# gk969/stm32-speech-recognition

Hardware: AMD Instinct MI355X
Metric: utterances/sec (256-frame, 100 templates) (higher is better)
Workload: dtype int32

## Files before the change

include/sr_engine.h:

```cpp
#ifndef SR_ENGINE_H
#define SR_ENGINE_H

#include <stddef.h>
#include <stdint.h>

#ifdef __cplusplus
extern "C" {
#endif

#define SR_OK 0
#define SR_ERR_NO_DEVICE 1
#define SR_ERR_BAD_CONFIG 2
#define SR_ERR_BAD_ARG 3
#define SR_ERR_NO_TEMPLATES 4
#define SR_ERR_HIP 5

#define SR_ST_OK 0
#define SR_ST_VAD_FAIL 1
#define SR_ST_MFCC_FAIL 2
#define SR_ST_SEG_OOB 3

#define SR_DIS_ERR 0xFFFFFFFFu
#define SR_SAVE_MASK 12345u

// ... 35 lines not shown

typedef struct sr_engine sr_engine;

void sr_default_config(sr_config *cfg);
int sr_create(const sr_config *cfg, sr_engine **out);
void sr_destroy(sr_engine *h);
const char *sr_last_error(void);

typedef struct sr_tables {
    uint16_t *hamm;
    uint16_t *tri_cen;
    uint16_t *tri_even;
    uint16_t *tri_odd;
    int8_t *dct;
    int16_t *tw_kr;
    int16_t *tw_ki;
    uint32_t *log_thr;
} sr_tables;
int sr_build_tables(const sr_config *cfg, const sr_tables *out);
int sr_build_tie_table(int8_t *out);
int sr_log_table_mismatches(void);
uint32_t sr_mag_cheap_bound(const sr_engine *h);
uint32_t sr_mag_table(uint16_t *out, uint32_t n);

int sr_set_templates(sr_engine *h, const void *store, uint32_t n_slots, uint32_t stride_bytes);
int sr_set_templates_dense(sr_engine *h, const int16_t *mfcc, const uint32_t *frames, const uint8_t *valid,
                           uint32_t n_templates, uint32_t tpl_stride);
uint32_t sr_num_templates(const sr_engine *h);
int sr_train_store(sr_engine *h, const uint16_t *pcm, uint64_t pcm_stride, uint32_t buf_len, uint32_t n,
                   const uint32_t *slot, void *store, uint32_t n_slots, uint32_t stride_bytes, uint32_t *status);

int sr_recognize_batch(sr_engine *h, const uint16_t *pcm, uint64_t pcm_stride, uint32_t buf_len, uint32_t B,
                       sr_result *results, uint32_t *scores, int16_t *mfcc, sr_vad_rec *vad);
int sr_recognize_batch_dev(sr_engine *h, const uint16_t *d_pcm, uint64_t pcm_stride, uint32_t buf_len, uint32_t B,
                           sr_result *d_results, uint32_t *d_scores, int16_t *d_mfcc, sr_vad_rec *d_vad,
                           void *stream);
int sr_recognize_batch_packed12(sr_engine *h, const uint8_t *packed, uint64_t row_stride_bytes, uint32_t buf_len, uint32_t B,
                                sr_result *results, uint32_t *scores, int16_t *mfcc, sr_vad_rec *vad);

int sr_recognize_segments_batch(sr_engine *h, const uint16_t *pcm, uint64_t pcm_stride, uint32_t buf_len, uint32_t B,
                                sr_result *results, uint32_t *scores, sr_vad_rec *vad);
int sr_recognize_segments_batch_dev(sr_engine *h, const uint16_t *d_pcm, uint64_t pcm_stride, uint32_t buf_len,
                                    uint32_t B, sr_result *d_results, uint32_t *d_scores, sr_vad_rec *d_vad,
                                    void *stream);

typedef struct sr_stream_seg {
// ... 242 lines not shown
```

stm32_speech_recognition_amd/csrc/k_mfcc.hip:

```cpp
#include "sr_fft_dev.h"

#include <type_traits>

#ifndef SR_MEL_CHUNKED
#define SR_MEL_CHUNKED 1
#endif

namespace sr {

constexpr int kMfccWaves = 4;
constexpr int kFramesPerWave = 16, kFramesPerWaveMid = 4, kFramesPerWaveSmall = 1;
#ifndef SR_MAG_TAB_BINS
#define SR_MAG_TAB_BINS 8
#endif
constexpr int mfcc_tab_bins(int fpw) { return fpw == kFramesPerWave ? SR_MAG_TAB_BINS : 0; }
static_assert(SR_MAG_TAB_BINS == 0 || SR_MAG_TAB_BINS == 4 || SR_MAG_TAB_BINS == 8, "table bins per lane");
#ifndef SR_MFCC_PIPE
#define SR_MFCC_PIPE 1
#endif
#ifndef SR_MFCC_PIPE_PEEL
#define SR_MFCC_PIPE_PEEL 1
#endif
#ifndef SR_MFCC_PIPE_VMCNT
#define SR_MFCC_PIPE_VMCNT (SR_MFCC_PIPE_PEEL ? 3 : 0)
#endif
static_assert(SR_MFCC_PIPE_VMCNT == 0 || (SR_MFCC_PIPE_VMCNT == 3 && SR_MFCC_PIPE_PEEL), "younger loads counted by the wait");
constexpr bool mfcc_pipelined(int fpw) { return SR_MFCC_PIPE && mfcc_tab_bins(fpw) == 8; }
constexpr int kMelPad = kMel + 1;
__device__ __forceinline__ constexpr int mel_chunk_word(int j) { return 256 * ((j >> 2) & 1) + 4 * ((j >> 3) ^ (4 * ((j >> 2) & 1))) + (j & 3); }
constexpr int mfcc_wave_lds_words(int fpw) { return kXchgWords + fpw * kMelPad + 64; }

template <typename Base>
struct MfccTabArgs : Base {
    const uint16_t *mag_q;
    uint32_t mag_table_off;
};
template <typename Base>
constexpr int mfcc_feat_kind<MfccTabArgs<Base>> = mfcc_feat_kind<Base>;
template <typename Base>
static MfccTabArgs<Base> mfcc_tab_args(const Base &b, const MfccMagTab &tab)
{
    MfccTabArgs<Base> r;
    static_cast<Base &>(r) = b;
    r.mag_q = tab.mag_q;
    r.mag_table_off = tab.mag_table_off;
    return r;
}

template <int kFPW, typename Args = MfccTabArgs<MfccArgs>>
__global__ void __launch_bounds__(64 * kMfccWaves, 4) k_mfcc(const Args a)
{
    constexpr int kFeat = mfcc_feat_kind<Args>;
    constexpr uint32_t kFeatW = (kFeat == SR_FEAT_FFT || kFeat == SR_FEAT_MAG) ? kBins : kMel;
    constexpr int kWaveLdsWords = mfcc_wave_lds_words(kFPW);
    constexpr int kTabBins = mfcc_tab_bins(kFPW);
    constexpr bool kPipe = mfcc_pipelined(kFPW);
    extern __shared__ __attribute__((aligned(16))) uint32_t smem[];
    __shared__ uint32_t s_dctM[kCoef * kMelPad];
    __shared__ int s_dctS[kCoef * kMelPad];
    __shared__ u32x4 s_tw3[kTw3Row * 4], s_tw5[8 * 64];
    __shared__ u32x4 s_tm[4 * 64];
    const int lane = threadIdx.x & 63, w = __builtin_amdgcn_readfirstlane(threadIdx.x >> 6);
    uint32_t *buf = smem + w * kWaveLdsWords;
    uint32_t *xw = buf;
    uint32_t *powb = buf + kXchgWords, *moff = powb + kFPW * kMelPad;

    for (int i = threadIdx.x; i < kCoef * kMel; i += blockDim.x) {
        const int c = a.t.dct[i], o = (i / kMel) * kMelPad + i % kMel;
        s_dctM[o] = (uint32_t)(((c < 0 ? -c : c) * 262144 + 99) / 100);
        s_dctS[o] = (c > 0) - (c < 0);
    }
    __syncthreads();

    LaneTw tw;
    load_lane_tw(a.t, lane, tw);
    if (w == 0 && lane < 4) {
        const uint32_t *f = &tw.s3[0][0][0];
#pragma unroll
        for (int c = 0; c < 8; c++) s_tw3[lane * kTw3Row + c] = u32x4{f[4 * c], f[4 * c + 1], f[4 * c + 2], f[4 * c + 3]};
    }
    if (w == 1 % kMfccWaves) store_tw32(s_tw5, lane, tw.s5);
#ifndef SR_INJECT_LDS_RACE
    if (w == 2 % kMfccWaves) {
#pragma unroll
        for (int c = 0; c < 2; c++) {
            s_tm[64 * c + lane] = *(const u32x4 *)(a.t.tri_even_m + 8 * lane + 4 * c);
            s_tm[64 * (c + 2) + lane] = *(const u32x4 *)(a.t.tri_odd_m + 8 * lane + 4 * c);
        }
    }
#endif
    __syncthreads();
#ifdef SR_INJECT_LDS_RACE
    if (w == 2 % kMfccWaves) {
#if SR_INJECT_LDS_RACE >= 2
        __builtin_amdgcn_s_sleep(127);
#endif
#pragma unroll
        for (int c = 0; c < 2; c++) {
            s_tm[64 * c + lane] = *(const u32x4 *)(a.t.tri_even_m + 8 * lane + 4 * c);
            s_tm[64 * (c + 2) + lane] = *(const u32x4 *)(a.t.tri_odd_m + 8 * lane + 4 * c);
        }
    }
#endif
    int hamm_m[3];
#pragma unroll
    for (int k = 0; k < 3; k++) hamm_m[k] = (lane + 64 * k < kFrameLen) ? hamm_fused_multiplier(a.t.hamm[lane + 64 * k]) : 0;
    int f_lo = 0, p_hi = 0, p_lo = 0, x_hi = 0, x_lo = 0;
    if (lane < kMel) {
        const int h = lane;
        f_lo = (h == 0) ? 0 : (int)a.t.tri_cen[h - 1];
        const int f_hi = (h == kMel - 1) ? kBins : (int)a.t.tri_cen[h + 1];
        const int ih = f_hi - 1, il = f_lo ? f_lo - 1 : 0, half = (h & 1) ? kBins : 0;
#if SR_MEL_CHUNKED
        p_hi = half + mel_chunk_word(ih), x_hi = (ih >> 3) > 0 ? (ih >> 3) - 1 : 0;
        p_lo = half + mel_chunk_word(il), x_lo = (il >> 3) > 0 ? (il >> 3) - 1 : 0;
#else
        p_hi = half + ih, x_hi = (ih >> 3) > 0 ? (ih >> 3) - 1 : 0;
        p_lo = half + il, x_lo = (il >> 3) > 0 ? (il >> 3) - 1 : 0;
#endif
    }
    const uint64_t mag_p = (uint64_t)a.mag_q;
    const u32x4 mag_rs = {(uint32_t)mag_p, (uint32_t)(mag_p >> 32) | (2u << 16), kMagTabEntries, 0x00027000u};
    const uint32_t tw_off = 32u * (uint32_t)lane;
#if SR_MEL_CHUNKED
    const int e_base = mel_chunk_word(lane);
    constexpr int kEs = 32, kEh = 128;
    const int c0 = mel_chunk_word(8 * lane), c1 = mel_chunk_word(8 * lane + 4);
#else
    const int e_base = lane;
    constexpr int kEs = 64, kEh = 256;
    const int c0 = 8 * lane, c1 = 8 * lane + 4;
#endif

    uint32_t item = blockIdx.x;
    uint32_t nx_nfrm = 0;
    int nx_mid = 0, nx_seg0 = 0;
    if (item < a.n_items) {
        const sr_vad_rec *rec = a.vad + item / a.tiles;
        nx_nfrm = rec->frm_num;
        nx_mid = (int)rec->atap.mid_val;
        nx_seg0 = rec->seg[0];
    }
    for (; item < a.n_items; item += gridDim.x) {
        const uint32_t b = item / a.tiles, tile = item - b * a.tiles;
        const uint32_t nfrm = nx_nfrm;
        const int mid = nx_mid, seg0 = nx_seg0;
        if (item + gridDim.x < a.n_items) {
            const sr_vad_rec *rec = a.vad + (item + gridDim.x) / a.tiles;
            nx_nfrm = rec->frm_num;
            nx_mid = (int)rec->atap.mid_val;
            nx_seg0 = rec->seg[0];
        }
        const uint16_t *row = a.pcm + (uint64_t)b * a.pcm_stride;
        int16_t *out = a.mfcc + (uint64_t)b * a.max_frames * kCoef;
        const uint32_t f0 = tile * (kMfccWaves * kFPW) + w * kFPW;
        uint32_t *frow = nullptr;
        if constexpr (kFeat != 0) frow = a.feat + (uint64_t)b * a.max_frames * kFeatW;
        uint32_t nf = 0;
        if (f0 < nfrm) nf = (nfrm - f0 < (uint32_t)kFPW) ? nfrm - f0 : (uint32_t)kFPW;

        uint32_t s_pp[3] = {0, 0, 0};
        if (nf) {
            const uint16_t *x = row + seg0 + (int)kHop * (int)f0;
#pragma unroll
            for (int k = 0; k < 3; k++) {
                const int i = lane + 64 * k;
                if (i < kFrameLen) s_pp[k] = *(const u32_align2 *)(x + i - 1);
            }
        }
        if constexpr (!kPipe)
        for (uint32_t fi = 0; fi < nf; fi++) {
#pragma unroll
            for (int k = 0; k < 3; k++) {
                const int i = lane + 64 * k;
                if (i < kFrameLen) xw[i] = k == 0 ? window_sample<4>(s_pp[k], mid, hamm_m[k]) : window_sample<2>(s_pp[k], mid, hamm_m[k]);
            }
            if (fi + 1 < nf) {
                const uint16_t *x = row + seg0 + (int)kHop * (int)(f0 + fi + 1);
#pragma unroll
                for (int k = 0; k < 3; k++) {
                    const int i = lane + 64 * k;
                    if (i < kFrameLen) s_pp[k] = *(const u32_align2 *)(x + i - 1);
// ... 288 lines not shown
                *(uint4 *)(buf + kBins + c0) = make_uint4(po[0], po[1], po[2], po[3]);
                *(uint4 *)(buf + kBins + c1) = make_uint4(po[4], po[5], po[6], po[7]);
                buf[2 * kBins + lane] = xe;
                moff[lane] = xo;
                wave_sync();
                if (lane < kMel) {
                    const uint32_t *X = (lane & 1) ? moff : buf + 2 * kBins;
                    const uint32_t hi = buf[p_hi] + X[x_hi], lo = f_lo ? buf[p_lo] + X[x_lo] : 0u;
                    powb[r * kMelPad + lane] = hi - lo;
                    if constexpr (kFeat == SR_FEAT_MEL) frow[(f0 + r) * kFeatW + lane] = hi - lo;
                }
                wave_sync();
            };
            constexpr std::false_type kDrain{};
            if (nf) {
                window();
                if (nf > 1) request(1);
#if SR_MFCC_PIPE_PEEL
                constexpr std::integral_constant<bool, SR_MFCC_PIPE_VMCNT != 0> kSteady{};
                {
                    wave_sync();
                    uint32_t v[4][4];
                    fft_front_real160(xw, lane, tw, s_tw3, v);
                    middle(0, v, nf > 1);
                }
                for (uint32_t fi = 1; fi + 1 < nf; fi++) {
                    wave_sync();
                    uint32_t v[4][4];
                    fft_front_real160(xw, lane, tw, s_tw3, v);
                    back_end(fi - 1, kSteady);
                    middle(fi, v, true);
                }
                if (nf > 1) {
                    wave_sync();
                    uint32_t v[4][4];
                    fft_front_real160(xw, lane, tw, s_tw3, v);
                    back_end(nf - 2, kDrain);
                    middle(nf - 1, v, false);
                }
#else
                for (uint32_t fi = 0; fi < nf; fi++) {
                    wave_sync();
                    uint32_t v[4][4];
                    fft_front_real160(xw, lane, tw, s_tw3, v);
                    if (fi > 0) back_end(fi - 1, kDrain);
                    middle(fi, v, fi + 1 < nf);
// ... 27 lines not shown
            for (uint32_t t = lane; t < nf * kFeatW; t += 64) {
                const uint32_t fi = t / kFeatW, h = t - fi * kFeatW;
                fw[t] = powb[fi * kMelPad + h] >> 14;
            }
        }
        {
            int16_t *out_w = out + (size_t)f0 * kCoef;
#pragma unroll
            for (uint32_t tl = lane; tl < (uint32_t)(kFPW * kCoef); tl += 64) {
                uint32_t t = tl;
                if constexpr (kPipe) asm volatile("" : "+v"(t));
                if (t < nf * kCoef) {
                    const uint32_t fi = umul24(t, 10923u) >> 17, h = t - umul24(fi, (uint32_t)kCoef);
                    const uint32_t *pw = powb + umul24(fi, (uint32_t)kMelPad), *dm = s_dctM + umul24(h, (uint32_t)kMelPad);
                    const int *ds = s_dctS + umul24(h, (uint32_t)kMelPad);
                    int acc = 0;
#pragma unroll
                    for (int i = 0; i < kMel; i++) acc = mad24((int)__umulhi(pw[i], dm[i]), ds[i], acc);
                    out_w[t] = (int16_t)acc;
                }
            }
        }
        wave_sync();
        {
            const uint32_t r0 = f0 + nf, r1 = (f0 + kFPW < a.max_frames) ? f0 + kFPW : a.max_frames;
            for (uint32_t t = r0 * kCoef + lane; t < r1 * kCoef && r0 < r1; t += 64) out[t] = 0;
        }
        if constexpr (kFeat != 0) {
            const uint32_t r0 = f0 + nf, r1 = (f0 + kFPW < a.max_frames) ? f0 + kFPW : a.max_frames;
            for (uint32_t t = r0 * kFeatW + lane; t < r1 * kFeatW && r0 < r1; t += 64) frow[t] = 0;
        }
    }
}

uint32_t mfcc_ext_frames_per_tile();
int mfcc_ext_occupancy(int *per_cu);
void launch_mfcc_ext(const MfccArgs &a, uint32_t grid, hipStream_t s);
void launch_mfcc_ext_features(const MfccArgs &a, int kind, uint32_t *feat, uint32_t grid, hipStream_t s);

uint32_t mfcc_frames_per_tile(uint32_t frame_len) { return frame_len == 320 ? mfcc_ext_frames_per_tile() : (uint32_t)(kMfccWaves * kFramesPerWave); }
uint32_t mfcc_frames_per_tile_small(uint32_t frame_len, uint32_t which)
{
    return frame_len == 320 ? mfcc_ext_frames_per_tile() : (uint32_t)(kMfccWaves * (which ? kFramesPerWaveSmall : kFramesPerWaveMid));
}

uint32_t mfcc_resident_workgroups(uint32_t frame_len)
{
    int dev = 0, n_cu = 0, per_cu = 0;
    if (hipGetDevice(&dev) != hipSuccess) return 0;
    if (hipDeviceGetAttribute(&n_cu, hipDeviceAttributeMultiprocessorCount, dev) != hipSuccess || n_cu < 1) return 0;
    int e;
    if (frame_len == 320)
        e = mfcc_ext_occupancy(&per_cu);
    else
// ... 73 lines not shown
```

stm32_speech_recognition_amd/csrc/sr_device.h:

```cpp
#pragma once
#include <hip/hip_runtime.h>

#include <cstdint>

#include "../../include/sr_engine.h"

namespace sr {

enum DevHook {
    kHookDtwU,
    kHookDtwTieG,
    kHookDtwKc,
    kHookMfccGrid,
    kHookPerturbLogThr,
    kHookLogThrFromHost,
    kHookMultiAllowDup,
    kHookDtwDebug,
    kHookCellsLiteral,
    kHookMagCheapOff,
    kHookMagTableOff,
    kHookStreamTile,
    kHookSpotChunk,
    kHookAlignPairs,
    kHookAlignGlobal,
// ... 131 lines not shown
void launch_live_scan(const LiveArgs &a, bool sad, hipStream_t s);
void launch_live_records(const LiveRecArgs &a, uint32_t n, hipStream_t s);

struct MfccArgs {
    const uint16_t *pcm;
    uint64_t pcm_stride;
    uint32_t B;
    uint32_t max_frames;
    const sr_vad_rec *vad;
    int16_t *mfcc;
    uint32_t tiles;
    uint32_t small_tiles;
    uint32_t n_items;
    uint32_t grid_cap;
    uint32_t mag_cheap_max;
    uint32_t frame_len;
    uint32_t generic;
    uint32_t hop, n_mel, n_coef;
    DevTables t;
};
struct MfccMagTab {
    const uint16_t *mag_q;
    uint32_t mag_table_off;
};

template <int kKind>
struct MfccFeatArgs : MfccArgs {
    uint32_t *feat;
};
template <typename Args>
constexpr int mfcc_feat_kind = 0;
template <int kKind>
constexpr int mfcc_feat_kind<MfccFeatArgs<kKind>> = kKind;
template <int kKind>
inline MfccFeatArgs<kKind> mfcc_feat_args(const MfccArgs &a, uint32_t *feat)
{
    MfccFeatArgs<kKind> f;
    static_cast<MfccArgs &>(f) = a;
    f.feat = feat;
    return f;
}

struct DtwArgs {
    const int16_t *mfcc;
    const sr_vad_rec *vad;
    const uint32_t *in_frames;
// ... 161 lines not shown
```

stm32_speech_recognition_amd/csrc/sr_engine.cpp:

```cpp
#include "sr_engine_internal.h"

#include <atomic>
#include <cstdio>
#include <cstdlib>

namespace sr {

static thread_local std::string g_err;
int set_error(int code, const std::string &msg)
{
    g_err = msg;
    return code;
}

#ifdef SR_TESTING
static std::atomic<int64_t> g_hooks[kHookCount];
int64_t dev_hook(DevHook h) { return g_hooks[h].load(std::memory_order_relaxed); }
static const char *const kHookNames[kHookCount] = {"dtw_u", "dtw_tie_g", "dtw_kc", "mfcc_grid", "perturb_log_thr",
                                                   "log_thr_from_host", "multi_allow_dup", "dtw_debug", "cells_literal",
                                                   "mag_cheap_off", "mag_table_off", "stream_tile_frames", "spot_chunk_cols",
                                                   "align_pairs", "align_marks_global"};
#endif
}

// ... 59 lines not shown
extern "C++" int sr::config_framing(const sr_config *cfg, ConfigFraming *out)
{
    FrontEnd fe;
    if (int rc = front_end_of(cfg, &fe)) return rc;
    if (cfg->max_frames < 2 || cfg->max_frames > 16383) return fail(SR_ERR_BAD_CONFIG, "max_frames must be 2..16383");
    const uint32_t noise_len = (cfg->fs / 1000) * cfg->noise_len_ms, atap_frm = (cfg->fs / 1000) * 30;
    if (noise_len == 0 || noise_len % atap_frm != 0 || noise_len % (uint32_t)fe.frame_len != 0)
        return fail(SR_ERR_BAD_CONFIG, "noise_len_ms: the noise head must be a non-zero multiple of the 30 ms block of noise_atap and of the frame length");
    const uint32_t step = cfg->frame_time_ms - cfg->frame_mov_ms;
    if (80 / step < 1 || 110 / step < 1) return fail(SR_ERR_BAD_CONFIG, "frame_time_ms - frame_mov_ms must not exceed 80 ms (VAD.C:72-75)");
    *out = ConfigFraming{(uint32_t)fe.frame_len, (uint32_t)fe.hop, 80 / step, 110 / step, noise_len, cfg->max_frames};
    return SR_OK;
}

int sr_log_table_mismatches(void) { return log_table_mismatches(); }
uint32_t sr_mag_cheap_bound(const sr_engine *h) { return h ? h->mag_cheap_max : 0u; }

uint32_t sr_mag_table(uint16_t *out, uint32_t n)
{
    std::vector<uint16_t> t;
    gen_mag_q(t);
    if (out) std::memcpy(out, t.data(), std::min<size_t>(n, t.size()) * 2);
    return (uint32_t)t.size();
}

int sr_testing_build(void)
{
#ifdef SR_TESTING
    return 1;
#else
    return 0;
#endif
}

int sr_dev_hook(const char *name, int64_t value)
{
    if (!name) return fail(SR_ERR_BAD_ARG, "null hook name");
#ifdef SR_TESTING
    for (int i = 0; i < kHookCount; i++)
        if (std::strcmp(name, kHookNames[i]) == 0) {
            g_hooks[i].store(value, std::memory_order_relaxed);
            return SR_OK;
        }
    return fail(SR_ERR_BAD_ARG, std::string("unknown development hook: ") + name);
#else
    (void)value;
// ... 116 lines not shown
            delete h;
            return fail(SR_ERR_HIP, std::string("hipFuncSetAttribute(") + kernel + ", MaxDynamicSharedMemorySize): " + hipGetErrorString(hipGetLastError()));
        }
    }
    build_tables(h->host, fe);
    warn_log_table();
    const HostTables &t = h->host;
    std::vector<uint32_t> te32(t.tri_even.begin(), t.tri_even.end()), to32(t.tri_odd.begin(), t.tri_odd.end());
    std::vector<uint32_t> tem(t.tri_even.size()), tom(t.tri_odd.size());
    for (size_t i = 0; i < tem.size(); i++) {
        if (t.tri_even[i] > kMelTriMax || t.tri_odd[i] > kMelTriMax) {
            delete h;
            return fail(SR_ERR_BAD_CONFIG, "internal: Mel triangle weight above the fused multiplier's range");
        }
        tem[i] = mel_fused_multiplier(t.tri_even[i]);
        tom[i] = mel_fused_multiplier(t.tri_odd[i]);
    }
    if (!h->generic && h->frame_len == (uint32_t)kFrameLen && (t.tri_cen.empty() || t.tri_cen[0] < 9)) {
        delete h;
        return fail(SR_ERR_BAD_CONFIG, "internal: first Mel centre below bin 9");
    }
    std::vector<uint32_t> hpk(t.hamm.size() / 2);
    for (size_t i = 0; i < hpk.size(); i++) hpk[i] = (uint32_t)t.hamm[2 * i] | ((uint32_t)t.hamm[2 * i + 1] << 16);
    struct Part {
        const void *src;
        size_t bytes;
        size_t off;
    } parts[17] = {{t.hamm.data(), t.hamm.size() * 2, 0},       {t.tri_even.data(), t.tri_even.size() * 2, 0},
                  {t.tri_odd.data(), t.tri_odd.size() * 2, 0}, {t.tri_cen.data(), t.tri_cen.size() * 2, 0},
                  {t.dct.data(), t.dct.size(), 0},             {t.tw_a.data(), t.tw_a.size() * 4, 0},
                  {t.tw_b.data(), t.tw_b.size() * 4, 0},       {t.log_thr.data(), t.log_thr.size() * 4, 0},
                  {t.w512_a.data(), t.w512_a.size() * 4, 0},   {t.w512_b.data(), t.w512_b.size() * 4, 0},
                  {te32.data(), te32.size() * 4, 0},           {to32.data(), to32.size() * 4, 0},
                  {t.tie_delta.data(), t.tie_delta.size(), 0}, {hpk.data(), hpk.size() * 4, 0},
                  {tem.data(), tem.size() * 4, 0},             {tom.data(), tom.size() * 4, 0},
                  {t.mag_q.data(), t.mag_q.size() * 2, 0}};
    if (t.tie_delta.size() != (size_t)kTieMax) {
        delete h;
        return fail(SR_ERR_BAD_CONFIG, "internal: DTW tie-threshold table does not fit 8 bits");
    }
    size_t total = 0;
    for (auto &p : parts) {
        p.off = total;
        total += (p.bytes + 255) & ~(size_t)255;
    }
    std::vector<uint8_t> blob(total, 0);
    for (auto &p : parts) std::memcpy(blob.data() + p.off, p.src, p.bytes);
    hipError_t e = hipMalloc(&h->table_blob, total);
    if (e == hipSuccess) e = hipMemcpy(h->table_blob, blob.data(), total, hipMemcpyHostToDevice);
    if (e != hipSuccess) {
        delete h;
        return fail(SR_ERR_HIP, std::string("table upload: ") + hipGetErrorString(e));
    }
    uint8_t *base = (uint8_t *)h->table_blob;
    h->dev.hamm = (const uint16_t *)(base + parts[0].off);
    h->dev.tri_even = (const uint16_t *)(base + parts[1].off);
    h->dev.tri_odd = (const uint16_t *)(base + parts[2].off);
    h->dev.tri_cen = (const uint16_t *)(base + parts[3].off);
    h->dev.dct = (const int8_t *)(base + parts[4].off);
    h->dev.tw_a = (const uint32_t *)(base + parts[5].off);
    h->dev.tw_b = (const uint32_t *)(base + parts[6].off);
    h->dev.log_thr = (const uint32_t *)(base + parts[7].off);
    h->dev.w512_a = (const uint32_t *)(base + parts[8].off);
    h->dev.w512_b = (const uint32_t *)(base + parts[9].off);
    h->dev.tri_even32 = (const uint32_t *)(base + parts[10].off);
    h->dev.tri_odd32 = (const uint32_t *)(base + parts[11].off);
    h->dev.tie_delta = (const int8_t *)(base + parts[12].off);
    h->dev.hamm_pk = (const uint32_t *)(base + parts[13].off);
    h->dev.tri_even_m = (const uint32_t *)(base + parts[14].off);
    h->dev.tri_odd_m = (const uint32_t *)(base + parts[15].off);
    h->dev_mag_q = (const uint16_t *)(base + parts[16].off);
    if (!h->generic && h->frame_len == (uint32_t)kFrameLen) {
        uint32_t *sw = nullptr;
        const uint32_t init[4] = {0, 0, 0xFFFFFFFFu, 0};
        uint32_t back[4] = {1, 0, 0, 0};
        hipError_t se = hipMalloc(&sw, sizeof init);
        if (se == hipSuccess) se = hipMemcpy(sw, init, sizeof init, hipMemcpyHostToDevice);
        if (se == hipSuccess) {
            launch_mag_fast_sweep(kMagCheapMax, (unsigned long long *)sw, sw + 2, nullptr);
            se = hipGetLastError();
        }
        if (se == hipSuccess) se = hipMemcpy(back, sw, sizeof back, hipMemcpyDeviceToHost);
        if (sw) (void)hipFree(sw);
        if (se != hipSuccess) {
            sr_destroy(h);
            return fail(SR_ERR_HIP, std::string("magnitude sweep: ") + hipGetErrorString(se));
        }
        const bool ok = back[0] == 0 && back[1] == 0;
        h->mag_cheap_max = ok ? kMagCheapMax : 0u;
        if (dev_hook(kHookMagCheapOff)) h->mag_cheap_max = 0;
        if (!ok) {
            char msg[160];
            std::snprintf(msg, sizeof msg, "sr_create: v_sqrt_f32 magnitude differs from the exact form at n = %u on this device; "
                          "every frame takes the exact root", back[2]);
// ... 306 lines not shown
```

stm32_speech_recognition_amd/csrc/sr_engine_internal.h:

```cpp
#pragma once
#include <hip/hip_runtime.h>

#include <algorithm>
#include <cstdint>
#include <cstring>
#include <string>
#include <vector>

#include "sr_device.h"
#include "sr_dtw_plan.h"
#include "sr_tables.h"

namespace sr {

int set_error(int code, const std::string &msg);
static inline int fail(int code, const std::string &msg) { return set_error(code, msg); }

#define HIP_TRY(expr)                                                                                  \
    do {                                                                                               \
        hipError_t e_ = (expr);                                                                        \
        if (e_ != hipSuccess)                                                                          \
            return fail(SR_ERR_HIP, std::string(#expr) + ": " + hipGetErrorString(e_));                \
    } while (0)

// ... 44 lines not shown
    }
};

template <typename T>
struct TmpDevBuf : DevBuf<T> {
    TmpDevBuf() = default;
    TmpDevBuf(const TmpDevBuf &) = delete;
    ~TmpDevBuf() { this->release(); }
};

}

using namespace sr;

static constexpr uint32_t kVadWideBelow = 1024, kMfccFill = 1024;
static constexpr uint32_t kPairCounters = 65536;

struct sr_engine {
    sr_config cfg;
    int device = 0;
    uint32_t noise_len = 0, atap_frm = 0;
    uint32_t n_cu = 256;
    LdsBudget lds;
    const uint16_t *dev_mag_q = nullptr;
    uint32_t mag_cheap_max = 0;
    uint32_t mfcc_tile = 64, mfcc_tile_mid = 64, mfcc_tile_small = 64, mfcc_grid_cap = 0;
    uint32_t frame_len = 160, hop = 80;
    uint32_t nc = 12, n_mel = 24;
    size_t mfcc_elems(size_t B) const { return B * cfg.max_frames * nc; }
    bool generic = false;
    uint32_t v_durmin = 8, s_durmax = 11;
    HostTables host;
    DevTables dev{};
    void *table_blob = nullptr;
    DevBuf<int16_t> tpl;
    DevBuf<uint32_t> tpl_frames;
    DevBuf<uint8_t> tpl_valid;
    bool tpl_staged_ok = true;
    DevBuf<uint32_t> tplR;
    DevBuf<uint32_t> tpl_frames_s, tpl_orig;
    DevBuf<uint32_t> tpl_rank;
    uint32_t K = 0, tpl_rows = 0, tpl_stride = 0;
    DtwPlan plan;
    uint32_t dp_lanes = 0;
    std::vector<uint32_t> cells_by_len;
    int small_launch = 0;
// ... 101 lines not shown
```

stm32_speech_recognition_amd/csrc/sr_fft_dev.h:

```cpp
#pragma once
#include "sr_dev.h"

namespace sr {

__device__ __forceinline__ void cxmul(uint32_t y, uint32_t ka, uint32_t kb, int &re, int &im)
{
    re = sdot2z(y, ka);
    im = sdot2z(y, kb);
}

template <int S>
__device__ __forceinline__ void r4_combine(int &ar, int &ai, int &br, int &bi, int &cr, int &ci, int &dr, int &di)
{
    int tr = cr + dr, ti = ci + di;
    dr = cr - dr;
    di = ci - di;
    cr = tr;
    ci = ti;
    ar >>= 2;
    ai >>= 2;
    ar += br >> (2 + S);
    ai += bi >> (2 + S);
    br = ar - (br >> (1 + S));
    bi = ai - (bi >> (1 + S));
// ... 85 lines not shown
    }
    k[3][0] = pk_sub(0u, k3[2][0]);
    k[3][1] = pk_sub(0u, k3[2][1]);
}

__device__ __forceinline__ void load_lane_tw(const DevTables &t, int lane, LaneTw &tw)
{
    const int d0 = lane & 3;
    {
        uint32_t k[3][2];
        load_tw3(t, 0, d0, k);
        tw.s2[0][0] = k[0][0];
        tw.s2[0][1] = k[0][1];
        tw.s2[1][0] = k[1][0];
        tw.s2[1][1] = k[1][1];
    }
#pragma unroll
    for (int d1 = 0; d1 < 4; d1++) load_tw4(t, 12, d0 + 4 * d1, tw.s3[d1]);
    load_tw4(t, 60, lane, tw.s4);
#pragma unroll
    for (int d3 = 0; d3 < 4; d3++) load_tw4(t, 252, lane + 64 * d3, tw.s5[d3]);
}

__device__ __forceinline__ void store_tw32(u32x4 *lds, int lane, const uint32_t (&k)[4][4][2])
{
    const uint32_t *f = &k[0][0][0];
#pragma unroll
    for (int c = 0; c < 8; c++) lds[c * 64 + lane] = u32x4{f[4 * c], f[4 * c + 1], f[4 * c + 2], f[4 * c + 3]};
}
__device__ __forceinline__ void load_tw32(const u32x4 *lds, int lane, uint32_t (&k)[4][4][2])
{
    uint32_t *f = &k[0][0][0];
#pragma unroll
    for (int c = 0; c < 8; c++) {
        const u32x4 q = lds[c * 64 + lane];
        f[4 * c] = q.x;
        f[4 * c + 1] = q.y;
        f[4 * c + 2] = q.z;
        f[4 * c + 3] = q.w;
    }
}
constexpr int kTw3Row = 9;
__device__ __forceinline__ void load_tw32_d0(const u32x4 *lds, int d0, uint32_t (&k)[4][4][2])
{
    uint32_t *f = &k[0][0][0];
#pragma unroll
    for (int c = 0; c < 8; c++) {
        const u32x4 q = lds[d0 * kTw3Row + c];
        f[4 * c] = q.x;
        f[4 * c + 1] = q.y;
        f[4 * c + 2] = q.z;
        f[4 * c + 3] = q.w;
    }
}

__device__ __forceinline__ void fft_front_real160(const uint32_t *xw, int lane, const LaneTw &tw, const u32x4 *tw3_lds,
                                                  uint32_t (&v)[4][4])
{
    const int d3 = (lane >> 2) & 3, d4 = lane >> 4;
    const int base = rev2(d4) + 4 * rev2(d3);
    uint32_t y[10];
#pragma unroll
    for (int m = 0; m < 10; m++) y[m] = *(const uint16_t *)(xw + base + 16 * m);
#pragma unroll
    for (int m = 0; m < 4; m++) asm("" : "+v"(y[m]));
// ... 92 lines not shown
```

stm32_speech_recognition_amd/csrc/sr_launch.cpp:

```cpp
#include "sr_engine_internal.h"

using namespace sr;
int check_batch(const sr_engine *h, uint32_t B)
{
    const uint32_t tile = std::min(h->mfcc_tile, std::min(h->mfcc_tile_mid, h->mfcc_tile_small));
    if ((uint64_t)B * ((h->cfg.max_frames + tile - 1) / tile) > 0xFFFFFFFFull) return fail(SR_ERR_BAD_ARG, "batch too large");
    return SR_OK;
}

int mark_scratch_user(sr_engine *h, hipStream_t s)
{
    if (!h->ev_scratch) HIP_TRY(hipEventCreateWithFlags(&h->ev_scratch, hipEventDisableTiming));
    HIP_TRY(hipEventRecord(h->ev_scratch, s));
    h->scratch_pending = true;
    return SR_OK;
}
int order_after_scratch_users(sr_engine *h, hipStream_t s)
{
    if (!h->scratch_pending) return SR_OK;
    if (hipEventQuery(h->ev_scratch) == hipSuccess) {
        h->scratch_pending = false;
        return SR_OK;
    }
    (void)hipGetLastError();
// ... 47 lines not shown
    if (h->mfcc_tile_small < h->mfcc_tile && h->small_launch != 1) {
        const uint32_t t_mid = (h->cfg.max_frames + h->mfcc_tile_mid - 1) / h->mfcc_tile_mid;
        const uint32_t t_small = (h->cfg.max_frames + h->mfcc_tile_small - 1) / h->mfcc_tile_small;
        if (h->small_launch == 2 || (uint64_t)B * t_mid < kMfccFill) {
            a.tiles = t_small;
            a.small_tiles = 2;
        } else if ((uint64_t)B * a.tiles < kMfccFill) {
            a.tiles = t_mid;
            a.small_tiles = 1;
        }
    }
    a.grid_cap = h->mfcc_grid_cap;
    a.mag_cheap_max = h->mag_cheap_max;
    a.frame_len = h->frame_len;
    a.n_items = B * a.tiles;
    a.generic = h->generic ? 1u : 0u;
    a.hop = h->hop;
    a.n_mel = h->n_mel;
    a.n_coef = h->nc;
    a.t = h->dev;
    return a;
}

MfccMagTab mfcc_mag_tab(const sr_engine *h) { return MfccMagTab{h->dev_mag_q, dev_hook(kHookMagTableOff) ? 1u : 0u}; }

int sr_mfcc_batch_dev(sr_engine *h, const uint16_t *d_pcm, uint64_t pcm_stride, uint32_t B, const sr_vad_rec *d_vad,
                      int16_t *d_mfcc, void *stream)
{
    if (!h || !d_pcm || !d_vad || !d_mfcc) return fail(SR_ERR_BAD_ARG, "null argument");
    if (pcm_stride >= (1ull << 31)) return fail(SR_ERR_BAD_ARG, "pcm_stride must be below 2^31 samples");
    if (int rcb = check_batch(h, B)) return rcb;
    ENTER_DEVICE(h);
    launch_mfcc(mfcc_args(h, d_pcm, pcm_stride, B, d_vad, d_mfcc), mfcc_mag_tab(h), (hipStream_t)stream);
    HIP_TRY(hipGetLastError());
    return SR_OK;
}

DtwArgs dtw_args(const sr_engine *h, const int16_t *d_mfcc, const sr_vad_rec *d_vad, const uint32_t *d_in_frames,
                        uint32_t B, uint32_t *d_scores, sr_result *d_results)
{
    DtwArgs a;
    a.mfcc = d_mfcc;
    a.vad = d_vad;
    a.in_frames = d_in_frames;
    a.B = B;
    a.max_frames = h->cfg.max_frames;
    a.tpl = h->tpl.p;
// ... 313 lines not shown
```

stm32_speech_recognition_amd/csrc/sr_tables.cpp:

```cpp
#include "sr_device.h"
#include "sr_tables.h"

#include <atomic>
#include <cmath>
#include <cstdio>
#include <cstdlib>

namespace sr {

static const uint32_t kLogThrRef[kLogMax + 2] = {
#include "sr_log_thr_ref.inc"
};
static std::atomic<int> g_log_mismatches{0};
int log_table_mismatches() { return g_log_mismatches.load(); }

static double mround(double v) { return v >= 0.0 ? std::floor(v + 0.5) : -std::floor(-v + 0.5); }

static void gen_hamm(HostTables &t, const FrontEnd &fe)
{
    t.hamm.resize(fe.frame_len);
    for (int i = 0; i < fe.frame_len; i++)
        t.hamm[i] = (uint16_t)mround((0.54 - 0.46 * std::cos(2 * M_PI * i / (fe.frame_len - 1))) * 10000.0);
}

// ... 111 lines not shown
}

static uint32_t root_u32(uint32_t d) { return (uint32_t)sqrtf((float)d); }

static void gen_tie_delta(HostTables &t)
{
    t.tie_delta.assign(kTieMax, 1);
    for (uint32_t g = 4095; g < (uint32_t)kTieMax; g++) {
        const uint64_t M = (uint64_t)(g + 1) * (g + 1);
        uint32_t d = (uint32_t)M;
        while (root_u32(d - 1) >= g + 1) d--;
        const int64_t delta = (int64_t)d - (int64_t)M + 1;
        t.tie_delta[g] = (int8_t)delta;
        if (delta < -128 || delta > 127) t.tie_delta.clear();
    }
}

void gen_mag_q(std::vector<uint16_t> &out)
{
    out.resize(kMagTabEntries);
    for (uint32_t n = 0; n < kMagTabEntries; n++) out[n] = (uint16_t)(((uint32_t)(sqrtf((float)n) * 10.0f)) << 2);
}

void build_tables(HostTables &t, const FrontEnd &fe)
{
    gen_mag_q(t.mag_q);
    gen_tie_delta(t);
    gen_hamm(t, fe);
    gen_tri(t, fe);
    gen_dct(t, fe);
    gen_twiddles(t);
    gen_log_thr(t);
    gen_w512(t);
}

}
```

stm32_speech_recognition_amd/csrc/sr_tables.h:

```cpp
#pragma once
#include <cstdint>
#include <vector>

namespace sr {

constexpr int kFrameLen = 160;
constexpr int kHop = 80;
constexpr int kNfft = 1024;
constexpr int kBins = 512;
constexpr int kMel = 24;
constexpr int kCoef = 12;
constexpr int kTwiddles = 1020;
constexpr int kLogMax = 2218;
constexpr int kTieMax = 32768;


constexpr int kWinShift = 5;
constexpr int32_t hamm_fused_multiplier(uint32_t h) { return (int32_t)((((uint64_t)h << 27) + 999u) / 1000u); }

constexpr uint32_t kMelFusedMaxE = (1u << 28) / 100u;
constexpr uint32_t kMagSmallMax = 26843;
static_assert(1638u * 1638u <= kMelFusedMaxE && 100ull * (kMagSmallMax + 1) < 1639ull * 1639ull, "quiet-frame bound");
constexpr uint32_t kMagCheapMax = 70171;
static_assert(kMagSmallMax <= kMagCheapMax, "the quiet tier lies inside the cheap-magnitude range");
// ... 3 lines not shown
constexpr uint32_t mel_fused_multiplier(uint32_t tri) { return (uint32_t)((((uint64_t)tri << 28) + 99u) / 100u); }

struct FrontEnd {
    int fs, frame_len, hop, nfft, bins, n_mel, n_coef;
    bool generic;
};
constexpr FrontEnd kFrontRef = {8000, 160, 80, 1024, 512, 24, 12, false};
constexpr FrontEnd kFrontExt = {16000, 320, 160, 512, 256, 40, 12, false};

struct HostTables {
    std::vector<uint16_t> hamm;
    std::vector<uint16_t> tri_cen;
    std::vector<uint16_t> tri_even;
    std::vector<uint16_t> tri_odd;
    std::vector<int8_t> dct;
    std::vector<uint32_t> tw_a, tw_b;
    std::vector<int16_t> tw_kr, tw_ki;
    std::vector<uint32_t> log_thr;
    std::vector<uint32_t> w512_a, w512_b;
    std::vector<int8_t> tie_delta;
    std::vector<uint16_t> mag_q;
};

void build_tables(HostTables &t, const FrontEnd &fe);
void gen_mag_q(std::vector<uint16_t> &out);
int log_table_mismatches();

}
```

Before: 3.299 million.

## Precompute per-lane MFCC constants into a packed image loaded with vector reads

Replaces the kernel prologue's scattered table loads and integer divisions (DCT magnitude/sign, twiddle gathers, hamming multipliers, mel edge offsets) with a host-built 16-byte-chunked image. Each wave copies its share into LDS, and each lane reads its own words with coalesced u32x4 loads. The per-tile zero-fill of padding rows moves ahead of compute so empty tiles can skip the body early. The cost is an extra device buffer and a duplicated layout contract between host and kernel.

Result: no change. 3.292 million (-0.2%).

```diff
diff --git a/include/sr_engine.h b/include/sr_engine.h
--- a/include/sr_engine.h
+++ b/include/sr_engine.h
@@ -81,6 +81,7 @@
 int sr_log_table_mismatches(void);
 uint32_t sr_mag_cheap_bound(const sr_engine *h);
 uint32_t sr_mag_table(uint16_t *out, uint32_t n);
+size_t sr_mfcc_lane_image(void *out, size_t bytes);
 
 int sr_set_templates(sr_engine *h, const void *store, uint32_t n_slots, uint32_t stride_bytes);
 int sr_set_templates_dense(sr_engine *h, const int16_t *mfcc, const uint32_t *frames, const uint8_t *valid,
diff --git a/stm32_speech_recognition_amd/csrc/k_mfcc.hip b/stm32_speech_recognition_amd/csrc/k_mfcc.hip
--- a/stm32_speech_recognition_amd/csrc/k_mfcc.hip
+++ b/stm32_speech_recognition_amd/csrc/k_mfcc.hip
@@ -1,10 +1,6 @@
 #include "sr_fft_dev.h"
 
 #include <type_traits>
-
-#ifndef SR_MEL_CHUNKED
-#define SR_MEL_CHUNKED 1
-#endif
 
 namespace sr {
 
@@ -26,14 +22,13 @@
 #endif
 static_assert(SR_MFCC_PIPE_VMCNT == 0 || (SR_MFCC_PIPE_VMCNT == 3 && SR_MFCC_PIPE_PEEL), "younger loads counted by the wait");
 constexpr bool mfcc_pipelined(int fpw) { return SR_MFCC_PIPE && mfcc_tab_bins(fpw) == 8; }
-constexpr int kMelPad = kMel + 1;
-__device__ __forceinline__ constexpr int mel_chunk_word(int j) { return 256 * ((j >> 2) & 1) + 4 * ((j >> 3) ^ (4 * ((j >> 2) & 1))) + (j & 3); }
 constexpr int mfcc_wave_lds_words(int fpw) { return kXchgWords + fpw * kMelPad + 64; }
 
 template <typename Base>
 struct MfccTabArgs : Base {
     const uint16_t *mag_q;
     uint32_t mag_table_off;
+    const u32x4 *lane_img;
 };
 template <typename Base>
 constexpr int mfcc_feat_kind<MfccTabArgs<Base>> = mfcc_feat_kind<Base>;
@@ -44,6 +39,7 @@
     static_cast<Base &>(r) = b;
     r.mag_q = tab.mag_q;
     r.mag_table_off = tab.mag_table_off;
+    r.lane_img = (const u32x4 *)tab.lane_img;
     return r;
 }
 
@@ -56,8 +52,8 @@
     constexpr int kTabBins = mfcc_tab_bins(kFPW);
     constexpr bool kPipe = mfcc_pipelined(kFPW);
     extern __shared__ __attribute__((aligned(16))) uint32_t smem[];
-    __shared__ uint32_t s_dctM[kCoef * kMelPad];
-    __shared__ int s_dctS[kCoef * kMelPad];
+    __shared__ __attribute__((aligned(16))) uint32_t s_dctM[kCoef * kMelPad];
+    __shared__ __attribute__((aligned(16))) int s_dctS[kCoef * kMelPad];
     __shared__ u32x4 s_tw3[kTw3Row * 4], s_tw5[8 * 64];
     __shared__ u32x4 s_tm[4 * 64];
     const int lane = threadIdx.x & 63, w = __builtin_amdgcn_readfirstlane(threadIdx.x >> 6);
@@ -65,71 +61,49 @@
     uint32_t *xw = buf;
     uint32_t *powb = buf + kXchgWords, *moff = powb + kFPW * kMelPad;
 
-    for (int i = threadIdx.x; i < kCoef * kMel; i += blockDim.x) {
-        const int c = a.t.dct[i], o = (i / kMel) * kMelPad + i % kMel;
-        s_dctM[o] = (uint32_t)(((c < 0 ? -c : c) * 262144 + 99) / 100);
-        s_dctS[o] = (c > 0) - (c < 0);
-    }
-    __syncthreads();
-
-    LaneTw tw;
-    load_lane_tw(a.t, lane, tw);
-    if (w == 0 && lane < 4) {
-        const uint32_t *f = &tw.s3[0][0][0];
-#pragma unroll
-        for (int c = 0; c < 8; c++) s_tw3[lane * kTw3Row + c] = u32x4{f[4 * c], f[4 * c + 1], f[4 * c + 2], f[4 * c + 3]};
-    }
-    if (w == 1 % kMfccWaves) store_tw32(s_tw5, lane, tw.s5);
+    const u32x4 *img = a.lane_img;
+    auto fill_tm = [&]() {
+#pragma unroll
+        for (int c = 0; c < 4; c++) s_tm[64 * c + lane] = img[kImgTm + 64 * c + lane];
+    };
+    auto fill_dct = [&](uint32_t *dst, int at) {
+        for (int c = lane; c < kImgDctChunks; c += 64) ((u32x4 *)dst)[c] = img[at + c];
+    };
+    if (w == 0) {
+        if (lane < kTw3Row * 4) s_tw3[lane] = img[kImgTw3 + lane];
+        fill_dct(s_dctM, kImgDctM);
+    }
+    if (w == 1 % kMfccWaves) {
+#pragma unroll
+        for (int c = 0; c < 8; c++) s_tw5[64 * c + lane] = img[kImgTw5 + 64 * c + lane];
+    }
 #ifndef SR_INJECT_LDS_RACE
-    if (w == 2 % kMfccWaves) {
-#pragma unroll
-        for (int c = 0; c < 2; c++) {
-            s_tm[64 * c + lane] = *(const u32x4 *)(a.t.tri_even_m + 8 * lane + 4 * c);
-            s_tm[64 * (c + 2) + lane] = *(const u32x4 *)(a.t.tri_odd_m + 8 * lane + 4 * c);
-        }
-    }
-#endif
+    if (w == 2 % kMfccWaves) fill_tm();
+#endif
+    if (w == 3 % kMfccWaves) fill_dct((uint32_t *)s_dctS, kImgDctS);
+    uint32_t lw[kLwCount];
+    load_lane_words(img, lane, lw);
     __syncthreads();
 #ifdef SR_INJECT_LDS_RACE
     if (w == 2 % kMfccWaves) {
 #if SR_INJECT_LDS_RACE >= 2
         __builtin_amdgcn_s_sleep(127);
 #endif
-#pragma unroll
-        for (int c = 0; c < 2; c++) {
-            s_tm[64 * c + lane] = *(const u32x4 *)(a.t.tri_even_m + 8 * lane + 4 * c);
-            s_tm[64 * (c + 2) + lane] = *(const u32x4 *)(a.t.tri_odd_m + 8 * lane + 4 * c);
-        }
-    }
-#endif
-    int hamm_m[3];
-#pragma unroll
-    for (int k = 0; k < 3; k++) hamm_m[k] = (lane + 64 * k < kFrameLen) ? hamm_fused_multiplier(a.t.hamm[lane + 64 * k]) : 0;
-    int f_lo = 0, p_hi = 0, p_lo = 0, x_hi = 0, x_lo = 0;
-    if (lane < kMel) {
-        const int h = lane;
-        f_lo = (h == 0) ? 0 : (int)a.t.tri_cen[h - 1];
-        const int f_hi = (h == kMel - 1) ? kBins : (int)a.t.tri_cen[h + 1];
-        const int ih = f_hi - 1, il = f_lo ? f_lo - 1 : 0, half = (h & 1) ? kBins : 0;
-#if SR_MEL_CHUNKED
-        p_hi = half + mel_chunk_word(ih), x_hi = (ih >> 3) > 0 ? (ih >> 3) - 1 : 0;
-        p_lo = half + mel_chunk_word(il), x_lo = (il >> 3) > 0 ? (il >> 3) - 1 : 0;
-#else
-        p_hi = half + ih, x_hi = (ih >> 3) > 0 ? (ih >> 3) - 1 : 0;
-        p_lo = half + il, x_lo = (il >> 3) > 0 ? (il >> 3) - 1 : 0;
-#endif
-    }
+        fill_tm();
+    }
+#endif
+    LaneTw tw;
+    lane_tw_from_words(lw, tw);
+    const int hamm_m[3] = {(int)lw[kLwHamm], (int)lw[kLwHamm + 1], (int)lw[kLwHamm + 2]};
+    const int f_lo = (int)lw[kLwFLo], p_hi = (int)lw[kLwPHi], p_lo = (int)lw[kLwPLo], x_hi = (int)lw[kLwXHi], x_lo = (int)lw[kLwXLo];
     const uint64_t mag_p = (uint64_t)a.mag_q;
     const u32x4 mag_rs = {(uint32_t)mag_p, (uint32_t)(mag_p >> 32) | (2u << 16), kMagTabEntries, 0x00027000u};
     const uint32_t tw_off = 32u * (uint32_t)lane;
+    const int e_base = (int)lw[kLwEBase], c0 = (int)lw[kLwC0], c1 = (int)lw[kLwC1];
 #if SR_MEL_CHUNKED
-    const int e_base = mel_chunk_word(lane);
     constexpr int kEs = 32, kEh = 128;
-    const int c0 = mel_chunk_word(8 * lane), c1 = mel_chunk_word(8 * lane + 4);
 #else
-    const int e_base = lane;
     constexpr int kEs = 64, kEh = 256;
-    const int c0 = 8 * lane, c1 = 8 * lane + 4;
 #endif
 
     uint32_t item = blockIdx.x;
@@ -158,6 +132,14 @@
         if constexpr (kFeat != 0) frow = a.feat + (uint64_t)b * a.max_frames * kFeatW;
         uint32_t nf = 0;
         if (f0 < nfrm) nf = (nfrm - f0 < (uint32_t)kFPW) ? nfrm - f0 : (uint32_t)kFPW;
+        {
+            const uint32_t r0 = f0 + nf, r1 = (f0 + kFPW < a.max_frames) ? f0 + kFPW : a.max_frames;
+            for (uint32_t t = r0 * kCoef + lane; t < r1 * kCoef && r0 < r1; t += 64) out[t] = 0;
+            if constexpr (kFeat != 0) {
+                for (uint32_t t = r0 * kFeatW + lane; t < r1 * kFeatW && r0 < r1; t += 64) frow[t] = 0;
+            }
+        }
+        if (nf == 0) continue;
 
         uint32_t s_pp[3] = {0, 0, 0};
         if (nf) {
@@ -492,6 +474,7 @@
                     wave_sync();
                     uint32_t v[4][4];
                     fft_front_real160(xw, lane, tw, s_tw3, v);
+                    asm volatile("" : "+v"(s_pp[0]), "+v"(s_pp[1]), "+v"(s_pp[2]));
                     middle(0, v, nf > 1);
                 }
                 for (uint32_t fi = 1; fi + 1 < nf; fi++) {
@@ -565,14 +548,6 @@
             }
         }
         wave_sync();
-        {
-            const uint32_t r0 = f0 + nf, r1 = (f0 + kFPW < a.max_frames) ? f0 + kFPW : a.max_frames;
-            for (uint32_t t = r0 * kCoef + lane; t < r1 * kCoef && r0 < r1; t += 64) out[t] = 0;
-        }
-        if constexpr (kFeat != 0) {
-            const uint32_t r0 = f0 + nf, r1 = (f0 + kFPW < a.max_frames) ? f0 + kFPW : a.max_frames;
-            for (uint32_t t = r0 * kFeatW + lane; t < r1 * kFeatW && r0 < r1; t += 64) frow[t] = 0;
-        }
     }
 }
 
diff --git a/stm32_speech_recognition_amd/csrc/sr_device.h b/stm32_speech_recognition_amd/csrc/sr_device.h
--- a/stm32_speech_recognition_amd/csrc/sr_device.h
+++ b/stm32_speech_recognition_amd/csrc/sr_device.h
@@ -177,6 +177,7 @@
 struct MfccMagTab {
     const uint16_t *mag_q;
     uint32_t mag_table_off;
+    const void *lane_img;
 };
 
 template <int kKind>
diff --git a/stm32_speech_recognition_amd/csrc/sr_engine.cpp b/stm32_speech_recognition_amd/csrc/sr_engine.cpp
--- a/stm32_speech_recognition_amd/csrc/sr_engine.cpp
+++ b/stm32_speech_recognition_amd/csrc/sr_engine.cpp
@@ -105,6 +105,16 @@
     gen_mag_q(t);
     if (out) std::memcpy(out, t.data(), std::min<size_t>(n, t.size()) * 2);
     return (uint32_t)t.size();
+}
+
+size_t sr_mfcc_lane_image(void *out, size_t bytes)
+{
+    HostTables t;
+    build_tables(t, kFrontRef);
+    std::vector<uint32_t> img;
+    build_mfcc_lane_image(t, img);
+    if (out) std::memcpy(out, img.data(), std::min(bytes, img.size() * 4));
+    return img.size() * 4;
 }
 
 int sr_testing_build(void)
@@ -267,11 +277,13 @@
     }
     std::vector<uint32_t> hpk(t.hamm.size() / 2);
     for (size_t i = 0; i < hpk.size(); i++) hpk[i] = (uint32_t)t.hamm[2 * i] | ((uint32_t)t.hamm[2 * i + 1] << 16);
+    std::vector<uint32_t> lane_img;
+    if (!h->generic && h->frame_len == (uint32_t)kFrameLen) build_mfcc_lane_image(t, lane_img);
     struct Part {
         const void *src;
         size_t bytes;
         size_t off;
-    } parts[17] = {{t.hamm.data(), t.hamm.size() * 2, 0},       {t.tri_even.data(), t.tri_even.size() * 2, 0},
+    } parts[18] = {{t.hamm.data(), t.hamm.size() * 2, 0},       {t.tri_even.data(), t.tri_even.size() * 2, 0},
                   {t.tri_odd.data(), t.tri_odd.size() * 2, 0}, {t.tri_cen.data(), t.tri_cen.size() * 2, 0},
                   {t.dct.data(), t.dct.size(), 0},             {t.tw_a.data(), t.tw_a.size() * 4, 0},
                   {t.tw_b.data(), t.tw_b.size() * 4, 0},       {t.log_thr.data(), t.log_thr.size() * 4, 0},
@@ -279,7 +291,7 @@
                   {te32.data(), te32.size() * 4, 0},           {to32.data(), to32.size() * 4, 0},
                   {t.tie_delta.data(), t.tie_delta.size(), 0}, {hpk.data(), hpk.size() * 4, 0},
                   {tem.data(), tem.size() * 4, 0},             {tom.data(), tom.size() * 4, 0},
-                  {t.mag_q.data(), t.mag_q.size() * 2, 0}};
+                  {t.mag_q.data(), t.mag_q.size() * 2, 0},     {lane_img.data(), lane_img.size() * 4, 0}};
     if (t.tie_delta.size() != (size_t)kTieMax) {
         delete h;
         return fail(SR_ERR_BAD_CONFIG, "internal: DTW tie-threshold table does not fit 8 bits");
@@ -315,6 +327,7 @@
     h->dev.tri_even_m = (const uint32_t *)(base + parts[14].off);
     h->dev.tri_odd_m = (const uint32_t *)(base + parts[15].off);
     h->dev_mag_q = (const uint16_t *)(base + parts[16].off);
+    if (!lane_img.empty()) h->dev_lane_img = base + parts[17].off;
     if (!h->generic && h->frame_len == (uint32_t)kFrameLen) {
         uint32_t *sw = nullptr;
         const uint32_t init[4] = {0, 0, 0xFFFFFFFFu, 0};
diff --git a/stm32_speech_recognition_amd/csrc/sr_engine_internal.h b/stm32_speech_recognition_amd/csrc/sr_engine_internal.h
--- a/stm32_speech_recognition_amd/csrc/sr_engine_internal.h
+++ b/stm32_speech_recognition_amd/csrc/sr_engine_internal.h
@@ -90,6 +90,7 @@
     uint32_t noise_len = 0, atap_frm = 0;
     uint32_t n_cu = 256;
     LdsBudget lds;
+    const void *dev_lane_img = nullptr;
     const uint16_t *dev_mag_q = nullptr;
     uint32_t mag_cheap_max = 0;
     uint32_t mfcc_tile = 64, mfcc_tile_mid = 64, mfcc_tile_small = 64, mfcc_grid_cap = 0;
diff --git a/stm32_speech_recognition_amd/csrc/sr_fft_dev.h b/stm32_speech_recognition_amd/csrc/sr_fft_dev.h
--- a/stm32_speech_recognition_amd/csrc/sr_fft_dev.h
+++ b/stm32_speech_recognition_amd/csrc/sr_fft_dev.h
@@ -131,6 +131,25 @@
     for (int d3 = 0; d3 < 4; d3++) load_tw4(t, 252, lane + 64 * d3, tw.s5[d3]);
 }
 
+__device__ __forceinline__ void load_lane_words(const u32x4 *img, int lane, uint32_t (&lw)[kLwCount])
+{
+#pragma unroll
+    for (int c = 0; c < kImgLaneChunks; c++) {
+        const u32x4 q = img[kImgLane + 64 * c + lane];
+        lw[4 * c] = q.x;
+        lw[4 * c + 1] = q.y;
+        lw[4 * c + 2] = q.z;
+        lw[4 * c + 3] = q.w;
+    }
+}
+__device__ __forceinline__ void lane_tw_from_words(const uint32_t (&lw)[kLwCount], LaneTw &tw)
+{
+#pragma unroll
+    for (int i = 0; i < 4; i++) tw.s2[i >> 1][i & 1] = lw[kLwS2 + i];
+#pragma unroll
+    for (int i = 0; i < 8; i++) tw.s4[i >> 1][i & 1] = lw[kLwS4 + i];
+}
+
 __device__ __forceinline__ void store_tw32(u32x4 *lds, int lane, const uint32_t (&k)[4][4][2])
 {
     const uint32_t *f = &k[0][0][0];
@@ -149,7 +168,6 @@
         f[4 * c + 3] = q.w;
     }
 }
-constexpr int kTw3Row = 9;
 __device__ __forceinline__ void load_tw32_d0(const u32x4 *lds, int d0, uint32_t (&k)[4][4][2])
 {
     uint32_t *f = &k[0][0][0];
diff --git a/stm32_speech_recognition_amd/csrc/sr_launch.cpp b/stm32_speech_recognition_amd/csrc/sr_launch.cpp
--- a/stm32_speech_recognition_amd/csrc/sr_launch.cpp
+++ b/stm32_speech_recognition_amd/csrc/sr_launch.cpp
@@ -93,7 +93,7 @@
     return a;
 }
 
-MfccMagTab mfcc_mag_tab(const sr_engine *h) { return MfccMagTab{h->dev_mag_q, dev_hook(kHookMagTableOff) ? 1u : 0u}; }
+MfccMagTab mfcc_mag_tab(const sr_engine *h) { return MfccMagTab{h->dev_mag_q, dev_hook(kHookMagTableOff) ? 1u : 0u, h->dev_lane_img}; }
 
 int sr_mfcc_batch_dev(sr_engine *h, const uint16_t *d_pcm, uint64_t pcm_stride, uint32_t B, const sr_vad_rec *d_vad,
                       int16_t *d_mfcc, void *stream)
diff --git a/stm32_speech_recognition_amd/csrc/sr_tables.cpp b/stm32_speech_recognition_amd/csrc/sr_tables.cpp
--- a/stm32_speech_recognition_amd/csrc/sr_tables.cpp
+++ b/stm32_speech_recognition_amd/csrc/sr_tables.cpp
@@ -157,6 +157,73 @@
     for (uint32_t n = 0; n < kMagTabEntries; n++) out[n] = (uint16_t)(((uint32_t)(sqrtf((float)n) * 10.0f)) << 2);
 }
 
+void build_mfcc_lane_image(const HostTables &t, std::vector<uint32_t> &img)
+{
+    img.assign((size_t)kImgChunks * 4, 0u);
+    auto chunk = [&](int c) { return img.data() + 4 * (size_t)c; };
+    auto pk_neg = [](uint32_t w) { return ((0u - w) & 0xFFFFu) | ((0u - (w >> 16)) << 16); };
+    auto tw4 = [&](int base, int b, uint32_t *k) {
+        const int e = base + 3 * b;
+        for (int leg = 0; leg < 3; leg++) {
+            k[2 * leg] = t.tw_a[e + 2 - leg];
+            k[2 * leg + 1] = t.tw_b[e + 2 - leg];
+        }
+        k[6] = pk_neg(k[4]);
+        k[7] = pk_neg(k[5]);
+    };
+    for (int lane = 0; lane < 64; lane++) {
+        uint32_t lw[kLwCount] = {};
+        uint32_t k[8];
+        tw4(0, lane & 3, k);
+        for (int i = 0; i < 4; i++) lw[kLwS2 + i] = k[i];
+        tw4(60, lane, lw + kLwS4);
+        for (int s = 0; s < 3; s++)
+            lw[kLwHamm + s] = (lane + 64 * s < kFrameLen) ? (uint32_t)hamm_fused_multiplier(t.hamm[lane + 64 * s]) : 0u;
+        if (lane < kMel) {
+            const int h = lane;
+            const int f_lo = (h == 0) ? 0 : (int)t.tri_cen[h - 1];
+            const int f_hi = (h == kMel - 1) ? kBins : (int)t.tri_cen[h + 1];
+            const int ih = f_hi - 1, il = f_lo ? f_lo - 1 : 0, half = (h & 1) ? kBins : 0;
+            lw[kLwFLo] = (uint32_t)f_lo;
+#if SR_MEL_CHUNKED
+            lw[kLwPHi] = (uint32_t)(half + mel_chunk_word(ih));
+            lw[kLwPLo] = (uint32_t)(half + mel_chunk_word(il));
+#else
+            lw[kLwPHi] = (uint32_t)(half + ih);
+            lw[kLwPLo] = (uint32_t)(half + il);
+#endif
+            lw[kLwXHi] = (uint32_t)((ih >> 3) > 0 ? (ih >> 3) - 1 : 0);
+            lw[kLwXLo] = (uint32_t)((il >> 3) > 0 ? (il >> 3) - 1 : 0);
+        }
+#if SR_MEL_CHUNKED
+        lw[kLwEBase] = (uint32_t)mel_chunk_word(lane);
+        lw[kLwC0] = (uint32_t)mel_chunk_word(8 * lane);
+        lw[kLwC1] = (uint32_t)mel_chunk_word(8 * lane + 4);
+#else
+        lw[kLwEBase] = (uint32_t)lane;
+        lw[kLwC0] = (uint32_t)(8 * lane);
+        lw[kLwC1] = (uint32_t)(8 * lane + 4);
+#endif
+        for (int c = 0; c < kImgLaneChunks; c++) std::copy(lw + 4 * c, lw + 4 * c + 4, chunk(kImgLane + 64 * c + lane));
+        uint32_t s5[32];
+        for (int d3 = 0; d3 < 4; d3++) tw4(252, lane + 64 * d3, s5 + 8 * d3);
+        for (int c = 0; c < 8; c++) std::copy(s5 + 4 * c, s5 + 4 * c + 4, chunk(kImgTw5 + 64 * c + lane));
+        for (int c = 0; c < 2; c++)
+            for (int i = 0; i < 4; i++) {
+                chunk(kImgTm + 64 * c + lane)[i] = mel_fused_multiplier(t.tri_even[8 * lane + 4 * c + i]);
+                chunk(kImgTm + 64 * (c + 2) + lane)[i] = mel_fused_multiplier(t.tri_odd[8 * lane + 4 * c + i]);
+            }
+    }
+    for (int d0 = 0; d0 < 4; d0++)
+        for (int d1 = 0; d1 < 4; d1++) tw4(12, d0 + 4 * d1, chunk(kImgTw3 + kTw3Row * d0 + 2 * d1));
+    uint32_t *dm = chunk(kImgDctM), *ds = chunk(kImgDctS);
+    for (int i = 0; i < kCoef * kMel; i++) {
+        const int c = t.dct[i], o = (i / kMel) * kMelPad + i % kMel;
+        dm[o] = (uint32_t)(((c < 0 ? -c : c) * 262144 + 99) / 100);
+        ds[o] = (uint32_t)((c > 0) - (c < 0));
+    }
+}
+
 void build_tables(HostTables &t, const FrontEnd &fe)
 {
     gen_mag_q(t.mag_q);
diff --git a/stm32_speech_recognition_amd/csrc/sr_tables.h b/stm32_speech_recognition_amd/csrc/sr_tables.h
--- a/stm32_speech_recognition_amd/csrc/sr_tables.h
+++ b/stm32_speech_recognition_amd/csrc/sr_tables.h
@@ -49,7 +49,36 @@
     std::vector<uint16_t> mag_q;
 };
 
+#ifndef SR_MEL_CHUNKED
+#define SR_MEL_CHUNKED 1
+#endif
+constexpr int kMelPad = kMel + 1;
+constexpr int kTw3Row = 9;
+constexpr int mel_chunk_word(int j) { return 256 * ((j >> 2) & 1) + 4 * ((j >> 3) ^ (4 * ((j >> 2) & 1))) + (j & 3); }
+enum MfccLaneWords {
+    kLwS2 = 0,
+    kLwS4 = 4,
+    kLwHamm = 12,
+    kLwFLo = 15,
+    kLwPHi = 16, kLwPLo = 17, kLwXHi = 18, kLwXLo = 19,
+    kLwEBase = 20,
+    kLwC0 = 21, kLwC1 = 22,
+    kLwCount = 24
+};
+constexpr int kImgLaneChunks = kLwCount / 4;
+constexpr int kImgDctChunks = kCoef * kMelPad / 4;
+static_assert(kCoef * kMelPad % 4 == 0, "DCT tables are whole 16-byte chunks");
+constexpr int kImgLane = 0;
+constexpr int kImgDctM = kImgLane + kImgLaneChunks * 64;
+constexpr int kImgDctS = kImgDctM + kImgDctChunks;
+constexpr int kImgTw3 = kImgDctS + kImgDctChunks;
+constexpr int kImgTw5 = kImgTw3 + kTw3Row * 4;
+constexpr int kImgTm = kImgTw5 + 8 * 64;
+constexpr int kImgChunks = kImgTm + 4 * 64;
+constexpr size_t kMfccLaneImageBytes = (size_t)kImgChunks * 16;
+
 void build_tables(HostTables &t, const FrontEnd &fe);
+void build_mfcc_lane_image(const HostTables &t, std::vector<uint32_t> &img);
 void gen_mag_q(std::vector<uint16_t> &out);
 int log_table_mismatches();
 
```
